# IBM/optimized-number-theoretic-transform-implementations

Measured on AMD Instinct MI355X. Metric: batched forward NTTs/sec at N=2^14, 50-bit q; achieved HBM GB/s vs peak, higher is better.
Workload: dtype f64

## Files before the change

### optimized-number-theoretic-transform-implementations_amd/csrc/ntt_arith.h

```cpp
#pragma once
#include <stdint.h>

#if defined(__HIPCC__)
#  include <hip/hip_runtime.h>
#  define NTT_HD __host__ __device__ __forceinline__
#  define NTT_DEVICE_CODE 1
#else
#  define NTT_HD inline __attribute__((always_inline))
#endif

namespace ntt {

struct alignas(16) TwU64 {
  uint64_t w;
  uint64_t con;
};
struct alignas(16) TwF64 {
  double w;
  double wq;
};

NTT_HD uint64_t mulhi64(uint64_t a, uint64_t b)
{
#if defined(__HIP_DEVICE_COMPILE__)
// ... 238 lines not shown
    const uint64_t p00 = a0 * b0, p01 = a0 * b1, p10 = a1 * b0, p11 = a1 * b1;
    const uint64_t mid = (p00 >> 32) + (uint32_t)p01 + (uint32_t)p10;
    lo                 = (uint32_t)p00 | (mid << 32);
    hi                 = p11 + (p01 >> 32) + (p10 >> 32) + (mid >> 32);
  }
  static NTT_HD uint64_t barrett(uint64_t hi, uint64_t lo, const consts &c)
  {
    const uint64_t q1 = (hi << (64u - c.bsh)) | (lo >> c.bsh);
    return lo - mulhi64(q1, c.bmu) * c.q;
  }
  static constexpr int kDotEvery = K == 3 ? 20 : (K == 1 ? 4 : 1);
  static constexpr int kDotChunk = 2;
  template <bool LAZY> static NTT_HD val dot_term(uint64_t a, uint64_t b, const consts &c)
  {
    if(LAZY && K <= 1) b = csub(b, c.q2);
    if(LAZY && K == 0) a = csub(a, c.q2);
    uint64_t hi, lo;
    mul128(a, b, hi, lo);
    return barrett(hi, lo, c);
  }
  static NTT_HD val dot_acc(val acc, val t, const consts &) { return acc + t; }
  static NTT_HD val dot_fold(val acc, const consts &c) { return reduce_any(acc, c); }
  template <bool LAZY> static NTT_HD val mul_out(val x, uint64_t b, const consts &c)
  {
    if(LAZY && K <= 1) b = csub(b, c.q2);
    if(LAZY && K == 0) b = csub(b, c.q);
    uint64_t hi, lo;
    mul128(reduce_any(x, c), b, hi, lo);
    return barrett(hi, lo, c);
  }
  static NTT_HD uint64_t mul_store(val r, const consts &c) { return csub(csub(r, c.q2), c.q); }
  static NTT_HD uint64_t mul_store_acc(val r, uint64_t acc, const consts &c) { return csub(csub(r + acc, c.q2), c.q); }
};

struct F64Consts {
  double q, qinv;
  double qinv_lo;
  double half_q;
  TwF64  ninv;
  TwF64  wninv;
  uint64_t qi;
  double   q2_sub;
};

struct ArithF64 {
  using val    = double;
  using tw     = TwF64;
  using consts = F64Consts;
  static constexpr bool kTracksBounds = true;
  static constexpr bool kCompact = true;
  static constexpr bool kRadix4  = false;
  static constexpr bool kWide52  = false;
  static constexpr bool kIntWide = false;
  using ctw                      = double;
  static NTT_HD tw expand(ctw w, const consts &c) { return tw{w, fma_(w, c.qinv, w * c.qinv_lo)}; }

  static NTT_HD double magic52() { return 4503599627370496.0; }

  static NTT_HD double u64_to_f64_lt52(uint64_t u)
  {
    union {
      uint64_t u;
      double   d;
    } x;
    x.u = u;
    return __builtin_ldexp(x.d, 1074);
  }
  static NTT_HD double reduce(double v, const consts &c)
  {
    const double k = rint_(v * c.qinv);
    return fma_(-k, c.q, v);
  }
  static NTT_HD double mulmod(const tw &t, double y, const consts &c)
  {
    const double h = y * t.w;
    const double k = rint_(y * t.wq);
    const double l = fma_(y, t.w, -h);
    const double d = fma_(-k, c.q, h);
    return d + l;
  }
  static NTT_HD double mulmod_c(ctw w, double y, const consts &c)
  {
    const double h = y * w;
    const double k = rint_(h * c.qinv);
    const double l = fma_(y, w, -h);
    const double d = fma_(-k, c.q, h);
    return d + l;
  }
  static NTT_HD double mulmod_c2(ctw w, double y, const consts &c)
  {
    const double h = y * w;
    const double k = rint_(fma_(h, c.qinv, h * c.qinv_lo));
    const double l = fma_(y, w, -h);
    const double d = fma_(-k, c.q, h);
    return d + l;
  }
  template <bool INV, bool WIDE> static NTT_HD val load(uint64_t raw, const consts &c)
  {
    if(WIDE) {
      raw = raw < 4 * c.qi ? raw : raw - 4 * c.qi;
      raw = raw < 2 * c.qi ? raw : raw - 2 * c.qi;
      raw = raw < c.qi ? raw : raw - c.qi;
    }
    return u64_to_f64_lt52(raw);
  }
  template <bool RED> static NTT_HD void fwd_bfly(val &x, val &y, const tw &t, const consts &c)
// ... 160 lines not shown
    const double s = x + y;
    const double d = y - x;
    x              = Base::reduce(s, c);
    y              = RED ? Base::mulmod_c(wneg, Base::reduce(d, c), c) : Base::mulmod_c2(wneg, d, c);
  }
  template <bool REDD, bool REDS> static NTT_HD void inv_bfly2(val &x, val &y, const tw &t, const consts &c)
  {
    const double s = x + y;
    const double d = x - y;
    x              = REDS ? Base::reduce(s, c) : s;
    y              = Base::mulmod(t, REDD ? Base::reduce(d, c) : d, c);
  }
  template <bool REDD, bool REDS> static NTT_HD void inv_bfly2(val &x, val &y, ctw w, const consts &c)
  {
    const double s = x + y;
    const double d = x - y;
    x              = REDS ? Base::reduce(s, c) : s;
    y              = REDD ? Base::mulmod_c(w, Base::reduce(d, c), c) : Base::mulmod_c2(w, d, c);
  }
  static NTT_HD void inv_bfly_last(val &x, val &y, const consts &c)
  {
    const double s = Base::reduce(x + y, c);
    const double d = Base::reduce(x - y, c);
    x              = Base::mulmod(c.ninv, s, c);
    y              = Base::mulmod(c.wninv, d, c);
  }
  static NTT_HD uint64_t store_fwd_lazy(val v, const consts &c) { return Base::store_fwd(v, c); }
  static constexpr int kDotEvery = 1;
  static constexpr int kDotChunk = 2;
  template <bool LAZY> static NTT_HD val dot_term(uint64_t a, uint64_t b, const consts &c)
  {
    if(LAZY) {
      a = a < 2 * c.qi ? a : a - 2 * c.qi;
      b = b < 2 * c.qi ? b : b - 2 * c.qi;
    }
    const double x0 = Base::u64_to_f64_lt52(a), y0 = Base::u64_to_f64_lt52(b);
    const double x  = Base::reduce(LAZY ? x0 - c.q : x0, c);
    const double y  = Base::reduce(LAZY ? y0 - c.q : y0, c);
    return Base::mulmod_c(y, x, c);
  }
};
using ArithF64W = WideF64<ArithF64>;

struct ArithF64S {
  using val    = double;
  using tw     = TwF64;
  using consts = F64Consts;
  using ctw    = double;
  static constexpr bool kTracksBounds = true;
  static constexpr bool kCompact      = true;
  static constexpr bool kRadix4       = false;
  static constexpr bool kWide52       = false;
  static constexpr bool kIntWide      = false;
  static NTT_HD tw expand(ctw w, const consts &c) { return ArithF64::expand(w, c); }

  static NTT_HD double word_to_val(uint64_t u)
  {
    union {
      uint64_t u;
      double   d;
    } x;
    x.u = u;
    return x.d;
  }
  static NTT_HD uint64_t val_to_word(double d)
  {
    union {
      double   d;
      uint64_t u;
    } x;
    x.d = d;
    return x.u;
  }
  static NTT_HD double reduce(double v, const consts &c)
  {
    const double k = v * c.qinv;
    return fma_(-k, c.q, v);
  }
  static NTT_HD double mulmod(const tw &t, double y, const consts &c)
  {
    const double h = y * t.w;
    const double k = y * t.wq;
    const double l = fma_(y, t.w, -h);
    const double d = fma_(-k, c.q, h);
    return d + l;
  }
  static NTT_HD double mulmod_c(ctw w, double y, const consts &c)
  {
    const double h = y * w;
    const double k = h * c.qinv;
    const double l = fma_(y, w, -h);
    const double d = fma_(-k, c.q, h);
    return d + l;
  }
  template <bool INV, bool WIDE> static NTT_HD val load(uint64_t raw, const consts &c)
  {
    if(WIDE) {
      raw = raw < 4 * c.qi ? raw : raw - 4 * c.qi;
      raw = raw < 2 * c.qi ? raw : raw - 2 * c.qi;
      raw = raw < c.qi ? raw : raw - c.qi;
    }
    return word_to_val(raw);
  }
  template <bool RED> static NTT_HD void fwd_bfly(val &x, val &y, const tw &t, const consts &c)
  {
    const double xr = RED ? reduce(x, c) : x;
    const double m  = mulmod(t, y, c);
    x               = xr + m;
    y               = xr - m;
  }
  template <bool RED> static NTT_HD void inv_bfly(val &x, val &y, const tw &t, const consts &c)
  {
    const double s = x + y;
    const double d = x - y;
    x              = RED ? reduce(s, c) : s;
    y              = mulmod(t, d, c);
  }
  template <bool RED> static NTT_HD void fwd_bfly(val &x, val &y, ctw w, const consts &c)
  {
    const double xr = RED ? reduce(x, c) : x;
    const double m  = mulmod_c(w, y, c);
    x               = xr + m;
    y               = xr - m;
  }
  template <bool RED> static NTT_HD void inv_bfly(val &x, val &y, ctw w, const consts &c)
  {
    const double s = x + y;
    const double d = x - y;
    x              = RED ? reduce(s, c) : s;
    y              = mulmod_c(w, d, c);
  }
  static NTT_HD void inv_bfly_last(val &x, val &y, const consts &c)
  {
    const double s = x + y;
    const double d = x - y;
    x              = mulmod(c.ninv, s, c);
    y              = mulmod(c.wninv, d, c);
  }
  static NTT_HD uint64_t to_canonical(double v, const consts &c)
  {
    const double   r = reduce(v, c);
    const uint64_t m = c.qi & (uint64_t)((int64_t)val_to_word(r) >> 63);
    return val_to_word(r + word_to_val(m));
  }
  static NTT_HD uint64_t store_fwd(val v, const consts &c) { return to_canonical(v, c); }
  static NTT_HD uint64_t store_inv(val v, const consts &c) { return to_canonical(v, c); }
  static NTT_HD uint64_t store_fwd_lazy(val v, const consts &c) { return val_to_word(v + c.q2_sub); }
  static NTT_HD uint64_t store_inv_lazy(val v, const consts &c) { return to_canonical(v, c); }
  static NTT_HD val      scale_ninv(val v, const consts &c) { return mulmod(c.ninv, v, c); }
};

template <class A> struct scaled_policy {
  using type = A;
};
template <> struct scaled_policy<ArithF64> {
  using type = ArithF64S;
};

struct F64Sched {
  uint32_t mask;
  double   bout;
};

constexpr double f64_rho(double b, double theta2) { return 0.5 + b * theta2 * 1.001 + 0.001; }

constexpr F64Sched f64_schedule_forced(bool inverse, int nstages, int ksh, double b_in, uint32_t cmask, uint32_t force);

constexpr F64Sched f64_schedule(bool inverse, int nstages, int ksh, double b_in, uint32_t cmask = 0, double bout_max = 1e30)
{
  uint32_t force = 0;
  F64Sched sc    = f64_schedule_forced(inverse, nstages, ksh, b_in, cmask, force);
  for(int s = nstages - 1; s >= 0 && sc.bout > bout_max; s--) {
    force |= 1u << s;
    sc = f64_schedule_forced(inverse, nstages, ksh, b_in, cmask, force);
  }
  return sc;
}

constexpr F64Sched f64_schedule_forced(bool inverse, int nstages, int ksh, double b_in, uint32_t cmask, uint32_t force)
{
  double theta2 = 0.25 * 1.001;
  double lim    = 4.0 / 1.001;
  for(int i = 0; i < ksh; i++) {
    theta2 *= 0.5;
    lim *= 2.0;
  }
  lim *= (1.0 - 1.0 / 64.0);
  double   b    = b_in;
  uint32_t mask = 0;
  const double theta2_full = theta2;
  for(int s = 0; s < nstages; s++) {
    theta2 = ((cmask >> s) & 1u) ? 1.5 * theta2_full : theta2_full;
    if(!inverse) {
      const double nr = b + f64_rho(b, theta2);
      if(nr > lim || ((force >> s) & 1u)) {
        mask |= (1u << s);
        b = 0.501 + f64_rho(b, theta2);
      } else {
        b = nr;
      }
    } else {
      const double two_b = 2.0 * b;
      const double r     = f64_rho(two_b, theta2);
      const double nr = two_b > r ? two_b : r;
      if(2.0 * nr > lim) {
        mask |= (1u << s);
        b = r > 0.501 ? r : 0.501;
      } else {
        b = nr;
      }
    }
  }
  return F64Sched{mask, b};
}

constexpr F64Sched f64w_fwd_schedule(int nstages, double b_in, uint32_t cmask)
{
  const double theta2 = 0.5;
  const double lim    = 2.0 * (1.0 - 1.0 / 64.0);
  double       b      = b_in;
  uint32_t     mask   = 0;
  for(int s = 0; s < nstages; s++) {
    const double cc   = ((cmask >> s) & 1u) ? 1.5 : 1.0;
    const double rho  = 0.5 + cc * b * theta2 * 1.001 + 0.001;
    const double ex   = rho + 0.5 * b * theta2 * 1.001;
    const double outb = 0.501 + rho;
    if(ex > lim || outb > lim || b > lim) {
      mask |= 1u << s;
      b = 0.501 + (0.5 + cc * 0.501 * theta2 * 1.001 + 0.001);
    } else {
      b = outb;
    }
  }
  return F64Sched{mask, b};
}

}
```

### optimized-number-theoretic-transform-implementations_amd/csrc/ntt_core.h

```cpp
#pragma once
#include <stdint.h>
#include <type_traits>
#include <utility>

#include "ntt_arith.h"
#include "ntt_passplan.h"

namespace ntt {

constexpr int kLE = 4;
constexpr int kE  = 1 << kLE;

template <int I, int N, class F> NTT_HD void static_for(F &&f)
{
  if constexpr(I < N) {
    f(std::integral_constant<int, I>{});
    static_for<I + 1, N>(f);
  }
}

constexpr int8_t kLaneBits[9][4][6] = {
   {{0, 1, -1, -1, -1, -1}, {2, 3, -1, -1, -1, -1}, {-1, -1, -1, -1, -1, -1}, {-1, -1, -1, -1, -1, -1}},
   {{0, 1, 2, -1, -1, -1}, {5, 6, 0, -1, -1, -1}, {1, 2, 3, -1, -1, -1}, {-1, -1, -1, -1, -1, -1}},
   {{0, 1, 2, 3, -1, -1}, {6, 7, 0, 1, -1, -1}, {2, 3, 4, 5, -1, -1}, {-1, -1, -1, -1, -1, -1}},
// ... 797 lines not shown
  const uint32_t ib = P::IBASE(G, t);
  static_assert(E0 % 2 == 0 && E1 % 2 == 0, "slots come in pairs");
  static_for<E0 / 2, E1 / 2>([&](auto hh) {
    constexpr int E = 2 * decltype(hh)::value;
    const u64x2   v = NT ? stream_load2_nt(coef_at(blk + P::IOFF(G, E), ib)) : stream_load2(coef_at(blk + P::IOFF(G, E), ib));
    raw[E]          = v.a;
    raw[E + 1]      = v.b;
  });
}

template <class A, int LOGN, bool INV>
NTT_HD void global_load_first(typename A::val (&x)[kE], uint32_t t, const uint64_t *blk,
                              bool wide, const typename A::consts &c)
{
  using P = Plan<LOGN>;
  uint64_t raw[kE];
  static_for<0, kE>([&](auto ee) {
    constexpr int   E   = decltype(ee)::value;
    const uint64_t *row = blk + ((uint32_t)E << P::LT);
    raw[E]              = stream_load(coef_at(row, t));
  });
  convert_inputs<A, INV>(x, raw, wide, c);
}

template <class A, int LOGN, bool INV>
NTT_HD void global_load_last(typename A::val (&x)[kE], uint32_t t, const uint64_t *blk,
                             bool wide, const typename A::consts &c)
{
  using P              = Plan<LOGN>;
  constexpr int G      = P::NG - 1;
  const uint32_t ib    = P::IBASE(G, t);
  uint64_t raw[kE];
  static_for<0, kE / 2>([&](auto hh) {
    constexpr int E = 2 * decltype(hh)::value;
    const u64x2   v = stream_load2(coef_at(blk + P::IOFF(G, E), ib));
    raw[E]          = v.a;
    raw[E + 1]      = v.b;
  });
  convert_inputs<A, INV>(x, raw, wide, c);
}

template <class A, bool INV, bool LAZYT> NTT_HD uint64_t out_word(typename A::val v, bool lazy_rt, const typename A::consts &c)
{
  if constexpr(A::kTracksBounds) {
    (void)lazy_rt;
    if constexpr(INV) return A::store_inv(v, c);
    else return LAZYT ? A::store_fwd_lazy(v, c) : A::store_fwd(v, c);
  } else {
    const uint64_t keep = lazy_rt ? 0ull : ~0ull;
    return INV ? A::store_inv_sel(v, c, keep) : A::store_fwd_sel(v, c, keep);
  }
}

template <class A, int LOGN, bool INV, bool LAZYT = false>
NTT_HD void global_store_first(const typename A::val (&x)[kE], uint32_t t, uint64_t *blk,
                               const typename A::consts &c, bool lazy_rt = false)
{
  using P = Plan<LOGN>;
  static_for<0, kE>([&](auto ee) {
    constexpr int E = decltype(ee)::value;
    stream_store(coef_at(blk + ((uint32_t)E << P::LT), t), out_word<A, INV, LAZYT>(x[E], lazy_rt, c));
  });
}

template <class A, int LOGN, bool INV, bool LAZYT = false>
NTT_HD void global_store_last(const typename A::val (&x)[kE], uint32_t t, uint64_t *blk,
                              const typename A::consts &c, bool lazy_rt = false)
{
  using P           = Plan<LOGN>;
  constexpr int G   = P::NG - 1;
  const uint32_t ib = P::IBASE(G, t);
  static_for<0, kE / 2>([&](auto hh) {
    constexpr int E = 2 * decltype(hh)::value;
    u64x2         v;
    v.a = out_word<A, INV, LAZYT>(x[E], lazy_rt, c);
    v.b = out_word<A, INV, LAZYT>(x[E + 1], lazy_rt, c);
    stream_store2(coef_at(blk + P::IOFF(G, E), ib), v);
  });
}

constexpr double kLazyBound = 1.99;

template <class A, int LOGN> constexpr uint32_t fused_cmask()
{
  using P        = Plan<LOGN>;
  uint32_t cmask = 0;
  for(int g = 0; g < P::NG; g++) {
    for(int j = 0; j < P::R(g); j++) {
      if(stage_is_compact<A, LOGN, false>(g, j)) cmask |= 1u << (P::S(g) + j);
    }
  }
  return cmask;
}

template <class A, int LOGN, bool INV, int KSH, bool LAZY = false> constexpr uint32_t fused_mask()
{
  if constexpr(A::kIntWide) {
    return u64x_schedule(INV, LOGN, A::kHead);
  } else if constexpr(!A::kTracksBounds) {
    return 0;
  } else {
    if constexpr(A::kWide52) {
      if constexpr(INV) return 0;
      else return f64w_fwd_schedule(LOGN, 1.0, 0u).mask;
    }
    if constexpr(INV) return kRedPlanFlag | (uint32_t)KSH;
    constexpr F64Sched sc = f64_schedule(false, LOGN, KSH, 1.0, fused_cmask<A, LOGN>(), LAZY ? kLazyBound : 1e30);
    static_assert(!LAZY || sc.bout <= kLazyBound, "lazy forward output: the reduction schedule cannot bound the last stage");
    return sc.mask;
  }
}

template <class A, int R, bool INV, uint32_t MASK>
NTT_HD void column_pass_thread(uint64_t *poly, uint32_t col, uint32_t logn, uint32_t S,
                               bool wide, bool lastinv, const typename A::tw *tab,
                               const typename A::consts &c, bool lazy_out = false)
{
  constexpr int  NE   = 1 << R;
  const uint32_t lsp  = logn - S - R;
  const uint32_t lo   = col & ((1u << lsp) - 1);
  const uint32_t hi   = col >> lsp;
  uint64_t *     base = poly + ((uint64_t)hi << (lsp + R)) + lo;
  typename A::val x[NE];
  static_for<0, NE>([&](auto ee) {
    constexpr int E = decltype(ee)::value;
    const uint64_t r = base[(uint64_t)E << lsp];
    x[E]             = wide ? A::template load<INV, true>(r, c) : A::template load<INV, false>(r, c);
  });
  static_for<0, R>([&](auto jj) {
    constexpr int  J   = INV ? (R - 1 - decltype(jj)::value) : decltype(jj)::value;
    constexpr int  AB  = R - 1 - J;
    constexpr int  POS = INV ? (R - 1 - J) : J;
    constexpr bool RED = (MASK >> POS) & 1u;
    const uint32_t tb  = (1u << (S + J)) + (hi << J);
    static_for<0, NE>([&](auto ee) {
      constexpr int E0 = decltype(ee)::value;
      if constexpr(((E0 >> AB) & 1) == 0) {
        constexpr int E1 = E0 | (1 << AB);
        if(INV && J == 0 && lastinv) {
          A::inv_bfly_last(x[E0], x[E1], c);
        } else {
          const typename A::tw w = tab[tb + (E0 >> (R - J))];
          if constexpr(INV) {
            A::template inv_bfly<RED>(x[E0], x[E1], w, c);
          } else {
            A::template fwd_bfly<RED>(x[E0], x[E1], w, c);
          }
        }
      }
    });
  });
  static_for<0, NE>([&](auto ee) {
    constexpr int E = decltype(ee)::value;
    base[(uint64_t)E << lsp] = out_word<A, INV, false>(x[E], lazy_out, c);
  });
}

template <class A, int R, bool INV>
NTT_HD void column_pass_thread_r4(uint64_t *poly, uint32_t col, uint32_t logn, uint32_t S, const typename A::tw *tab,
                                  const typename A::consts &c, bool lazy_out)
{
// ... 131 lines not shown
```

### optimized-number-theoretic-transform-implementations_amd/csrc/ntt_kernels_block.h

```cpp
#pragma once

namespace ntt {

__device__ __forceinline__ bool below(uint64_t a, uint64_t b) { return (int64_t)(a - b) < 0; }
constexpr int kPreAlso = 12;
constexpr int kIpreMin = 12;

template <class A> constexpr int flavor_of() { return A::kCompact ? 1 : (A::kRadix4 ? 2 : 0); }

template <int LOGN, bool INV, int FLAVOR> struct Geom {
  static constexpr bool COMPACT = FLAVOR == 1 || FLAVOR == 3;
  using P = Plan<LOGN>;
  static constexpr bool PERSIST2 = FLAVOR == 1 && LOGN == 13 && !INV;
  static constexpr int WG  = PERSIST2 ? 1024 : (P::T < 256 ? 256 : P::T);
  static constexpr int BPW = PERSIST2 ? 2 : (P::T < 256 ? 256 / P::T : 1);
  static constexpr bool PERSISTENT = BPW == 1 || PERSIST2;
  static constexpr bool group_is_per_lane(int g)
  {
    for(int j = 0; j < P::R(g); j++)
      if(P::TW_UNIFORM(g, j)) return false;
    return true;
  }
  static constexpr int TBL(int g)
  {
// ... 179 lines not shown
{
  typedef unsigned int v2u32 __attribute__((ext_vector_type(2)));
  const v2u32 v = __builtin_amdgcn_raw_buffer_load_b64(r, (int)voff, (int)soff, AUX);
  return (uint64_t)v.x | ((uint64_t)v.y << 32);
}
template <int AUX = kLoadAux> __device__ __forceinline__ u64x2 buffer_load_u64x2(__amdgpu_buffer_rsrc_t r, uint32_t voff, uint32_t soff)
{
  typedef unsigned int v4u32 __attribute__((ext_vector_type(4)));
  const v4u32 v = __builtin_amdgcn_raw_buffer_load_b128(r, (int)voff, (int)soff, AUX);
  return u64x2{(uint64_t)v.x | ((uint64_t)v.y << 32), (uint64_t)v.z | ((uint64_t)v.w << 32)};
}

template <int LOGN, int AUX = 0>
__device__ __forceinline__ void buffer_store_first_raw(const uint64_t (&u)[kE], uint32_t t, uint64_t *blk)
{
  using P                        = Plan<LOGN>;
  const __amdgpu_buffer_rsrc_t r = block_rsrc<LOGN>(blk);
  typedef unsigned int v2u32 __attribute__((ext_vector_type(2)));
  static_for<0, kE>([&](auto ee) {
    constexpr int E = decltype(ee)::value;
    v2u32         v;
    v.x = (unsigned)u[E];
    v.y = (unsigned)(u[E] >> 32);
    __builtin_amdgcn_raw_buffer_store_b64(v, r, (int)(t * 8u), (int)(((uint32_t)E << P::LT) * 8u), AUX);
  });
}

template <int LOGN, int AUX = kLoadAux>
__device__ __forceinline__ void prefetch_first(uint64_t (&raw)[kE], uint32_t t, const uint64_t *blk, bool live = true)
{
  using P = Plan<LOGN>;
  const __amdgpu_buffer_rsrc_t r = block_rsrc<LOGN>(blk, live);
  static_for<0, kE>([&](auto ee) {
    constexpr int E = decltype(ee)::value;
    raw[E]          = buffer_load_u64<AUX>(r, t * 8u, ((uint32_t)E << P::LT) * 8u);
  });
}

template <int LOGN, int AUX = kLoadAux>
__device__ __forceinline__ void prefetch_last(uint64_t (&raw)[kE], uint32_t t, const uint64_t *blk, bool live = true)
{
  using P           = Plan<LOGN>;
  constexpr int G   = P::NG - 1;
  const uint32_t ib = P::IBASE(G, t);
  const __amdgpu_buffer_rsrc_t r = block_rsrc<LOGN>(blk, live);
  static_for<0, kE / 2>([&](auto hh) {
    constexpr int E = 2 * decltype(hh)::value;
    const u64x2   v = buffer_load_u64x2<AUX>(r, ib * 8u, P::IOFF(G, E) * 8u);
    raw[E]          = v.a;
    raw[E + 1]      = v.b;
  });
}

template <class A, int LOGN, bool LAZYT, int AUX = 0>
__device__ __forceinline__ void store_last_whole_lines(const typename A::val (&x)[kE], uint32_t t, uint64_t *blk,
                                                       const typename A::consts &c, bool lazy_rt)
{
  using P          = Plan<LOGN>;
  constexpr int G  = P::NG - 1;
  constexpr int HB = P::TB(G, 5);
  static_assert(P::RL == 2 && P::NL == 6 && HB > 1, "needs runs of four coefficients per lane and full waves");
  uint64_t u[kE];
  static_for<0, kE>([&](auto ee) { u[decltype(ee)::value] = out_word<A, false, LAZYT>(x[decltype(ee)::value], lazy_rt, c); });
  static_for<0, kE>([&](auto ee) {
    constexpr int E = decltype(ee)::value;
    if constexpr((E & 2) == 0) {
      const auto lo = __builtin_amdgcn_permlane32_swap((unsigned)u[E], (unsigned)u[E | 2], false, false);
      const auto hi = __builtin_amdgcn_permlane32_swap((unsigned)(u[E] >> 32), (unsigned)(u[E | 2] >> 32), false, false);
      u[E]          = (uint64_t)lo[0] | ((uint64_t)hi[0] << 32);
      u[E | 2]      = (uint64_t)lo[1] | ((uint64_t)hi[1] << 32);
    }
  });
  const uint32_t ib   = (P::IBASE(G, t) & ~(1u << HB)) | (((t >> 5) & 1u) << 1);
  const __amdgpu_buffer_rsrc_t r = block_rsrc<LOGN>(blk);
  typedef unsigned int v4u32 __attribute__((ext_vector_type(4)));
  static_for<0, kE / 2>([&](auto hh) {
    constexpr int      E   = 2 * decltype(hh)::value;
    constexpr uint32_t OFF = (P::IOFF(G, E) & ~2u) | ((uint32_t)((E >> 1) & 1) << HB);
    v4u32              v;
    v.x = (unsigned)u[E];
    v.y = (unsigned)(u[E] >> 32);
    v.z = (unsigned)u[E + 1];
    v.w = (unsigned)(u[E + 1] >> 32);
    __builtin_amdgcn_raw_buffer_store_b128(v, r, (int)(ib * 8u), (int)(OFF * 8u), AUX);
  });
}

__device__ __forceinline__ void pin_raw(const uint64_t (&raw)[kE])
{
#pragma unroll
  for(int e = 0; e < kE; e++) asm volatile("" ::"v"(raw[e]));
}
template <class A, int LOGN, int G>
__device__ __forceinline__ void pin_preloaded(const typename A::ctw (&pre)[4][kE / 2])
{
  using P = Plan<LOGN>;
#pragma unroll
  for(int j = 0; j < P::R(G); j++) {
#pragma unroll
    for(int b = 0; b < kE / 2; b++) {
      if(P::BFLY_FIRST(G, j, b) == b) asm volatile("" ::"v"(pre[j][b]));
    }
  }
}

template <class A, int LOGN, bool INV, class G = Geom<LOGN, INV, flavor_of<A>()>>
__device__ __forceinline__ void fill_lds_tables(typename A::ctw *tabl, const Params<A> &p, uint32_t blk0, uint32_t tid)
{
  using P = Plan<LOGN>;
  static_for<0, P::NG>([&](auto gg) {
    constexpr int GI = decltype(gg)::value;
    if constexpr(G::TBL(GI) > 0) {
      typename A::ctw *tg = tabl + G::TBL_OFF(GI);
      static_for<0, P::R(GI)>([&](auto jj) {
        constexpr int JJ  = decltype(jj)::value;
        constexpr int SG  = P::S(GI);
        constexpr int SLJ = SG + JJ;
        const typename A::ctw *src = p.tw8 + ((size_t)1 << (p.s0 + SLJ)) + ((size_t)blk0 << SLJ);
        for(uint32_t l = tid; l < (1u << SLJ); l += G::WG) {
          const uint32_t u = l & ((1u << JJ) - 1u), prefix = l >> JJ;
          tg[(((1u << JJ) - 1u) << SG) + (u << SG) + prefix] = src[l];
        }
      });
    }
  });
}

template <class AK, int LOGN, bool INV, int KSH, bool LASTINV = false, bool LAZY = false, bool MULTI = false>
__global__ void __launch_bounds__((Geom<LOGN, INV, flavor_of<AK>()>::WG), (Geom<LOGN, INV, flavor_of<AK>()>::WPS)) fused_kernel(const KArgs<AK> k)
{
  using A = typename scaled_policy<AK>::type;
  uint32_t        bid, gdim, limb_;
  const Params<A> p = limb_params<A, INV, MULTI>(k, bid, gdim, limb_);
  using P                 = Plan<LOGN>;
  using G                 = Geom<LOGN, INV, flavor_of<A>()>;
  static_assert(!LAZY || (!INV && A::kTracksBounds), "the LAZY variant exists for the FP64 forward kernels only");
  constexpr uint32_t MASK = fused_mask<A, LOGN, INV, KSH, LAZY>() | (INV && LASTINV ? kLastInvFlag : 0u) | (INV && A::kWide52 ? kCanonInFlag : 0u);
  constexpr int LDS_TW = G::LDS_TW;
  __shared__ typename A::val lds_all[G::BPW * P::LDS_ELEMS + LDS_TW];

  const uint32_t     tid = threadIdx.x;
  const uint32_t     sub = G::PERSIST2 ? uniform_u32(tid >> P::LT) : (tid >> P::LT);
  const uint32_t     t   = tid & (P::T - 1);
  typename A::val *  lds = lds_all + sub * P::LDS_ELEMS;
  const uint32_t     bmask = (1u << p.s0) - 1u;

  if constexpr(!INV && G::PERSISTENT && !A::kRadix4) {
    constexpr int  GL     = P::NG - 1;
    constexpr bool PRE    = A::kCompact && (LOGN == 14 || LOGN == 13 || LOGN == kPreAlso) && stage_is_compact<A, LOGN, false>(GL, 0) && G::TBL(GL) == 0;
    constexpr bool LTW    = LDS_TW > 0;
    const uint32_t         tt     = G::BPW == 1 ? tid : t;
    typename A::val *const ll     = G::BPW == 1 ? lds_all : lds;
    const uint64_t         stride = (uint64_t)gdim * G::BPW;
    uint64_t               b0     = (uint64_t)bid * G::BPW;
    if(b0 >= p.nblocks) return;
    const uint64_t lastb = p.nblocks - 1;
    uint64_t       b     = G::BPW == 1 ? b0 : (b0 + sub < p.nblocks ? b0 + sub : lastb);
    typename A::ctw *const tabl = reinterpret_cast<typename A::ctw *>(lds_all + G::BPW * P::LDS_ELEMS);
    const lds_ctw_ptr<A>   ltw  = (lds_ctw_ptr<A>)tabl;
    if constexpr(LTW) {
      fill_lds_tables<A, LOGN, INV>(tabl, p, (uint32_t)b & bmask, tid);
      __syncthreads();
    }
    const auto next_blk = [&](uint64_t at) -> uint64_t {
      const uint64_t n0 = below(at + stride, p.nblocks) ? at + stride : at;
      return G::BPW == 1 ? n0 : (n0 + sub < p.nblocks ? n0 + sub : lastb);
    };
    uint64_t off_cur = blk_off_t<LOGN>(p, b), off_nxt = blk_off_t<LOGN>(p, next_blk(b0));
    uint64_t raw[kE];
    prefetch_first<LOGN>(raw, tt, p.a + off_cur);
    pin_raw(raw);
    typename A::ctw pre[4][kE / 2];
    if constexpr(PRE) {
      preload_group_tw<A, LOGN, GL>(pre, tt, (uint32_t)b & bmask, p);
      pin_preloaded<A, LOGN, GL>(pre);
    }
    for(; b0 < p.nblocks; b0 += stride) {
      const bool live = G::BPW == 1 || b0 + sub < p.nblocks;
      b               = live ? b0 + (G::BPW == 1 ? 0u : sub) : lastb;
      const uint32_t blk  = (uint32_t)b & bmask;
      uint64_t *     base = p.a + off_cur;
      typename A::val x[kE];
      convert_inputs<A, false>(x, raw, p.wide != 0, p.c);
      {
        const bool     more = b0 + stride < p.nblocks;
        prefetch_first<LOGN>(raw, tt, p.a + off_nxt, more);
        off_cur = off_nxt;
        off_nxt = blk_off_t<LOGN>(p, next_blk(more ? b0 + stride : b0));
      }
      run_group<A, LOGN, 0, false, MASK>(x, tt, blk, p);
      static_for<0, P::NG - 1>([&](auto gg) {
        constexpr int GI = decltype(gg)::value;
        exchange<A, LOGN, GI, GI + 1>(x, tt, ll);
        if constexpr(PRE && GI + 1 == GL) {
          run_group_preloaded<A, LOGN, GL, MASK>(x, pre, p);
        } else if constexpr(G::TBL(GI + 1) > 0) {
          run_group<A, LOGN, GI + 1, false, MASK, true>(x, tt, blk, p, ltw + G::TBL_OFF(GI + 1));
        } else {
          run_group<A, LOGN, GI + 1, false, MASK>(x, tt, blk, p);
        }
      });
      if constexpr(LOGN == 14) {
        store_last_whole_lines<A, LOGN, LAZY>(x, tid, base, p.c, p.lazy != 0);
      } else {
        if(live) global_store_last<A, LOGN, false, LAZY>(x, tt, base, p.c, p.lazy != 0);
      }
    }
    return;
  }
  if constexpr(INV && G::PERSISTENT && A::kCompact) {
    constexpr int  GL     = P::NG - 1;
    constexpr bool LTW    = LDS_TW > 0;
    const uint32_t         tt     = G::BPW == 1 ? tid : t;
    typename A::val *const ll     = G::BPW == 1 ? lds_all : lds;
    const uint64_t         stride = (uint64_t)gdim * G::BPW;
    uint64_t               b0     = (uint64_t)bid * G::BPW;
    if(b0 >= p.nblocks) return;
    const uint64_t lastb = p.nblocks - 1;
    uint64_t       b     = G::BPW == 1 ? b0 : (b0 + sub < p.nblocks ? b0 + sub : lastb);
    typename A::ctw *const tabl = reinterpret_cast<typename A::ctw *>(lds_all + G::BPW * P::LDS_ELEMS);
    const lds_ctw_ptr<A>   ltw  = (lds_ctw_ptr<A>)tabl;
    if constexpr(LTW) {
      fill_lds_tables<A, LOGN, INV>(tabl, p, (uint32_t)b & bmask, tid);
      __syncthreads();
    }
    constexpr bool IPRE = A::kCompact && LOGN >= kIpreMin && stage_is_compact<A, LOGN, true>(GL, 0) && P::R(GL) < 4 && G::TBL(GL) == 0 &&
                          !(LOGN == 12 && KSH == 1);
    typename A::ctw pre[4][kE / 2];
    if constexpr(IPRE) preload_group_tw<A, LOGN, GL>(pre, tt, (uint32_t)b & bmask, p);
    const auto next_blk = [&](uint64_t at) -> uint64_t {
      const uint64_t n0 = below(at + stride, p.nblocks) ? at + stride : at;
      return G::BPW == 1 ? n0 : (n0 + sub < p.nblocks ? n0 + sub : lastb);
    };
    uint64_t off_cur = blk_off_t<LOGN>(p, b), off_nxt = blk_off_t<LOGN>(p, next_blk(b0));
    uint64_t raw[kE];
    prefetch_last<LOGN>(raw, tt, p.a + off_cur);
    pin_raw(raw);
    if constexpr(IPRE) pin_preloaded<A, LOGN, GL>(pre);
    for(; b0 < p.nblocks; b0 += stride) {
      const bool live = G::BPW == 1 || b0 + sub < p.nblocks;
      b               = live ? b0 + (G::BPW == 1 ? 0u : sub) : lastb;
      const uint32_t blk  = (uint32_t)b & bmask;
      uint64_t *     base = p.a + off_cur;
      typename A::val x[kE];
      convert_inputs<A, true>(x, raw, p.wide != 0, p.c);
      {
        const bool     more = b0 + stride < p.nblocks;
        prefetch_last<LOGN>(raw, tt, p.a + off_nxt, more);
        off_cur = off_nxt;
        off_nxt = blk_off_t<LOGN>(p, next_blk(more ? b0 + stride : b0));
      }
      if constexpr(IPRE) {
        run_group_preloaded<A, LOGN, GL, MASK, true>(x, pre, p);
      } else if constexpr(G::TBL(GL) > 0) {
        run_group<A, LOGN, GL, true, MASK, true>(x, tt, blk, p, ltw + G::TBL_OFF(GL));
      } else {
        run_group<A, LOGN, GL, true, MASK>(x, tt, blk, p);
      }
      static_for<0, P::NG - 1>([&](auto gg) {
        constexpr int GI = P::NG - 1 - decltype(gg)::value;
        exchange<A, LOGN, GI, GI - 1>(x, tt, ll);
        if constexpr(G::TBL(GI - 1) > 0) {
          run_group<A, LOGN, GI - 1, true, MASK, true>(x, tt, blk, p, ltw + G::TBL_OFF(GI - 1));
        } else {
          run_group<A, LOGN, GI - 1, true, MASK>(x, tt, blk, p);
        }
      });
      uint64_t out[kE];
      static_for<0, kE>([&](auto ee) { out[decltype(ee)::value] = A::store_inv(x[decltype(ee)::value], p.c); });
      if(live) buffer_store_first_raw<LOGN>(out, tt, base);
    }
    return;
  }

  const lds_ctw_ptr<A> gtw = (lds_ctw_ptr<A>)reinterpret_cast<typename A::ctw *>(lds_all + G::BPW * P::LDS_ELEMS);
  if constexpr(LDS_TW > 0) {
    fill_lds_tables<A, LOGN, INV>(reinterpret_cast<typename A::ctw *>(lds_all + G::BPW * P::LDS_ELEMS), p, 0u, tid);
    __syncthreads();
  }
  for(uint64_t b0 = (uint64_t)bid * G::BPW; b0 < p.nblocks; b0 += (uint64_t)gdim * G::BPW) {
    uint64_t   b    = b0 + sub;
    const bool live = b < p.nblocks;
    if(!live) b = p.nblocks - 1;
    const uint32_t blk  = (uint32_t)b & bmask;
    uint64_t *     base = p.a + (poly_offset<false>(b >> p.s0, p.pstride, p.ptab) + ((b & bmask) << LOGN));
    typename A::val x[kE];
    if constexpr(!INV) {
      global_load_first<A, LOGN, false>(x, t, base, p.wide != 0, p.c);
      run_group<A, LOGN, 0, false, MASK, (G::TBL(0) > 0)>(x, t, blk, p, gtw);
      static_for<0, P::NG - 1>([&](auto gg) {
        constexpr int GI = decltype(gg)::value;
        exchange<A, LOGN, GI, GI + 1>(x, t, lds);
        run_group<A, LOGN, GI + 1, false, MASK, (G::TBL(GI + 1) > 0)>(x, t, blk, p, gtw + G::TBL_OFF(GI + 1));
      });
      if(live) global_store_last<A, LOGN, false, LAZY>(x, t, base, p.c, p.lazy != 0);
    } else {
      global_load_last<A, LOGN, true>(x, t, base, p.wide != 0, p.c);
      run_group<A, LOGN, P::NG - 1, true, MASK, (G::TBL(P::NG - 1) > 0)>(x, t, blk, p, gtw + G::TBL_OFF(P::NG - 1));
      static_for<0, P::NG - 1>([&](auto gg) {
        constexpr int GI = P::NG - 1 - decltype(gg)::value;
        exchange<A, LOGN, GI, GI - 1>(x, t, lds);
        run_group<A, LOGN, GI - 1, true, MASK, (G::TBL(GI - 1) > 0)>(x, t, blk, p, gtw + G::TBL_OFF(GI - 1));
      });
      if(live) global_store_first<A, LOGN, true>(x, t, base, p.c, p.lazy != 0);
    }
  }
}

template <int LEAD> __device__ __forceinline__ __amdgpu_buffer_rsrc_t poly_rsrc(const uint64_t *poly)
{
  return __builtin_amdgcn_make_buffer_rsrc(const_cast<uint64_t *>(poly), 0, (int)(8u << (kFusedLarge + LEAD)), 0x00020000);
}

template <class A, int LEAD, bool INV, int KSH>
__device__ __forceinline__ void twophase_columns(uint64_t *base, uint32_t tid, const Params<A> &p, bool wide_in, bool lazy_out)
{
  constexpr int      NE    = 1 << LEAD;
  constexpr int      CPR   = kE / NE;
  constexpr int      NR    = kE / CPR;
  constexpr uint32_t CMASK = column_mask<A, LEAD, INV, KSH>();
  const __amdgpu_buffer_rsrc_t r = poly_rsrc<LEAD>(base);
  typedef unsigned int v2u32 __attribute__((ext_vector_type(2)));
  uint64_t raw[kE];
  auto load_round = [&](auto rr, uint64_t(&dst)[kE]) {
    constexpr int RD = decltype(rr)::value;
    static_for<0, kE>([&](auto vv) {
      constexpr int      V   = decltype(vv)::value;
      constexpr uint32_t OFF = ((uint32_t)(V % NE) << kFusedLarge) + (uint32_t)(RD * CPR + V / NE) * 1024u;
      dst[V]                 = buffer_load_u64(r, tid * 8u, OFF * 8u);
    });
  };
  load_round(std::integral_constant<int, 0>{}, raw);
  static_for<0, NR>([&](auto rr) {
    constexpr int RD = decltype(rr)::value;
    typename A::val x[kE];
    convert_inputs<A, INV>(x, raw, wide_in, p.c);
    if constexpr(RD + 1 < NR) load_round(std::integral_constant<int, RD + 1>{}, raw);
    static_for<0, LEAD>([&](auto jj) {
      constexpr int  J   = INV ? (LEAD - 1 - decltype(jj)::value) : decltype(jj)::value;
      constexpr int  AB  = LEAD - 1 - J;
      constexpr int  POS = INV ? (LEAD - 1 - J) : J;
      constexpr bool RED = (CMASK >> POS) & 1u;
      static_for<0, kE>([&](auto vv) {
        constexpr int V  = decltype(vv)::value;
        constexpr int E0 = V % NE;
        if constexpr(((E0 >> AB) & 1) == 0) {
          constexpr int V1 = V | (1 << AB);
          if constexpr(INV && J == 0) {
// ... 391 lines not shown
```

Baseline: 19.92 million.

## Offset forward FP64 scaled outputs by half-q to drop final canonicalization select

For the scaled FP64 forward kernel, subtracts (q-1)/2 (in scaled representation) from coefficient 0 of the input. Since the NTT is linear, this shifts every output by that constant, so the final store can use a single reduce plus add of the offset instead of reduce, sign mask and conditional add. The reduction schedule gains per-policy constants (tighter for the scaled policy) and a relaxed output bound, which may remove intermediate reduction stages. This relies on the offset keeping results in [0,q) and on the bound analysis being correct.

```diff
diff --git a/optimized-number-theoretic-transform-implementations_amd/csrc/ntt_arith.h b/optimized-number-theoretic-transform-implementations_amd/csrc/ntt_arith.h
--- a/optimized-number-theoretic-transform-implementations_amd/csrc/ntt_arith.h
+++ b/optimized-number-theoretic-transform-implementations_amd/csrc/ntt_arith.h
@@ -314,6 +314,7 @@
   static constexpr bool kRadix4  = false;
   static constexpr bool kWide52  = false;
   static constexpr bool kIntWide = false;
+  static constexpr double kSchedFull = 1.0, kSchedCompact = 1.5;
   using ctw                      = double;
   static NTT_HD tw expand(ctw w, const consts &c) { return tw{w, fma_(w, c.qinv, w * c.qinv_lo)}; }
 
@@ -580,6 +581,7 @@
   static constexpr bool kRadix4       = false;
   static constexpr bool kWide52       = false;
   static constexpr bool kIntWide      = false;
+  static constexpr double kSchedFull = 0.5, kSchedCompact = 1.0;
   static NTT_HD tw expand(ctw w, const consts &c) { return ArithF64::expand(w, c); }
 
   static NTT_HD double word_to_val(uint64_t u)
@@ -673,6 +675,8 @@
   }
   static NTT_HD uint64_t store_fwd(val v, const consts &c) { return to_canonical(v, c); }
   static NTT_HD uint64_t store_inv(val v, const consts &c) { return to_canonical(v, c); }
+  static NTT_HD double   half_off(const consts &c) { return word_to_val((c.qi - 1u) >> 1); }
+  static NTT_HD uint64_t store_fwd_off(val v, double hoff, const consts &c) { return val_to_word(reduce(v, c) + hoff); }
   static NTT_HD uint64_t store_fwd_lazy(val v, const consts &c) { return val_to_word(v + c.q2_sub); }
   static NTT_HD uint64_t store_inv_lazy(val v, const consts &c) { return to_canonical(v, c); }
   static NTT_HD val      scale_ninv(val v, const consts &c) { return mulmod(c.ninv, v, c); }
@@ -692,20 +696,22 @@
 
 constexpr double f64_rho(double b, double theta2) { return 0.5 + b * theta2 * 1.001 + 0.001; }
 
-constexpr F64Sched f64_schedule_forced(bool inverse, int nstages, int ksh, double b_in, uint32_t cmask, uint32_t force);
-
-constexpr F64Sched f64_schedule(bool inverse, int nstages, int ksh, double b_in, uint32_t cmask = 0, double bout_max = 1e30)
+constexpr F64Sched f64_schedule_forced(bool inverse, int nstages, int ksh, double b_in, uint32_t cmask, uint32_t force, double cf = 1.0,
+                                       double cc = 1.5);
+
+constexpr F64Sched f64_schedule(bool inverse, int nstages, int ksh, double b_in, uint32_t cmask = 0, double bout_max = 1e30, double cf = 1.0,
+                                double cc = 1.5)
 {
   uint32_t force = 0;
-  F64Sched sc    = f64_schedule_forced(inverse, nstages, ksh, b_in, cmask, force);
+  F64Sched sc    = f64_schedule_forced(inverse, nstages, ksh, b_in, cmask, force, cf, cc);
   for(int s = nstages - 1; s >= 0 && sc.bout > bout_max; s--) {
     force |= 1u << s;
-    sc = f64_schedule_forced(inverse, nstages, ksh, b_in, cmask, force);
+    sc = f64_schedule_forced(inverse, nstages, ksh, b_in, cmask, force, cf, cc);
   }
   return sc;
 }
 
-constexpr F64Sched f64_schedule_forced(bool inverse, int nstages, int ksh, double b_in, uint32_t cmask, uint32_t force)
+constexpr F64Sched f64_schedule_forced(bool inverse, int nstages, int ksh, double b_in, uint32_t cmask, uint32_t force, double cf, double cc)
 {
   double theta2 = 0.25 * 1.001;
   double lim    = 4.0 / 1.001;
@@ -718,7 +724,7 @@
   uint32_t mask = 0;
   const double theta2_full = theta2;
   for(int s = 0; s < nstages; s++) {
-    theta2 = ((cmask >> s) & 1u) ? 1.5 * theta2_full : theta2_full;
+    theta2 = (((cmask >> s) & 1u) ? cc : cf) * theta2_full;
     if(!inverse) {
       const double nr = b + f64_rho(b, theta2);
       if(nr > lim || ((force >> s) & 1u)) {
diff --git a/optimized-number-theoretic-transform-implementations_amd/csrc/ntt_core.h b/optimized-number-theoretic-transform-implementations_amd/csrc/ntt_core.h
--- a/optimized-number-theoretic-transform-implementations_amd/csrc/ntt_core.h
+++ b/optimized-number-theoretic-transform-implementations_amd/csrc/ntt_core.h
@@ -873,6 +873,23 @@
   }
 }
 
+template <class A> NTT_HD void fwd_offset_input(typename A::val (&x)[kE], bool first, typename A::val hoff)
+{
+  if(first) x[0] = x[0] - hoff;
+}
+template <class A, bool INV, bool LAZYT, bool OFFS>
+NTT_HD uint64_t out_word_off(typename A::val v, bool lazy_rt, typename A::val hoff, const typename A::consts &c)
+{
+  if constexpr(OFFS) {
+    static_assert(!INV && !LAZYT, "offset outputs: the canonical forward output only");
+    (void)lazy_rt;
+    return A::store_fwd_off(v, hoff, c);
+  } else {
+    (void)hoff;
+    return out_word<A, INV, LAZYT>(v, lazy_rt, c);
+  }
+}
+
 template <class A, int LOGN, bool INV, bool LAZYT = false>
 NTT_HD void global_store_first(const typename A::val (&x)[kE], uint32_t t, uint64_t *blk,
                                const typename A::consts &c, bool lazy_rt = false)
@@ -884,9 +901,9 @@
   });
 }
 
-template <class A, int LOGN, bool INV, bool LAZYT = false>
+template <class A, int LOGN, bool INV, bool LAZYT = false, bool OFFS = false>
 NTT_HD void global_store_last(const typename A::val (&x)[kE], uint32_t t, uint64_t *blk,
-                              const typename A::consts &c, bool lazy_rt = false)
+                              const typename A::consts &c, bool lazy_rt = false, typename A::val hoff = {})
 {
   using P           = Plan<LOGN>;
   constexpr int G   = P::NG - 1;
@@ -894,8 +911,8 @@
   static_for<0, kE / 2>([&](auto hh) {
     constexpr int E = 2 * decltype(hh)::value;
     u64x2         v;
-    v.a = out_word<A, INV, LAZYT>(x[E], lazy_rt, c);
-    v.b = out_word<A, INV, LAZYT>(x[E + 1], lazy_rt, c);
+    v.a = out_word_off<A, INV, LAZYT, OFFS>(x[E], lazy_rt, hoff, c);
+    v.b = out_word_off<A, INV, LAZYT, OFFS>(x[E + 1], lazy_rt, hoff, c);
     stream_store2(coef_at(blk + P::IOFF(G, E), ib), v);
   });
 }
@@ -914,8 +931,9 @@
   return cmask;
 }
 
-template <class A, int LOGN, bool INV, int KSH, bool LAZY = false> constexpr uint32_t fused_mask()
-{
+template <class A, int LOGN, bool INV, int KSH, bool LAZY = false, bool OFFS = false> constexpr uint32_t fused_mask()
+{
+  static_assert(!OFFS || (!INV && !LAZY && A::kTracksBounds && !A::kWide52), "offset outputs: the canonical forward output of the FP64 policy");
   if constexpr(A::kIntWide) {
     return u64x_schedule(INV, LOGN, A::kHead);
   } else if constexpr(!A::kTracksBounds) {
@@ -926,8 +944,10 @@
       else return f64w_fwd_schedule(LOGN, 1.0, 0u).mask;
     }
     if constexpr(INV) return kRedPlanFlag | (uint32_t)KSH;
-    constexpr F64Sched sc = f64_schedule(false, LOGN, KSH, 1.0, fused_cmask<A, LOGN>(), LAZY ? kLazyBound : 1e30);
+    constexpr double   bmax = LAZY ? kLazyBound : (OFFS ? kLazyBound * (double)(1u << (KSH < 31 ? KSH : 31)) : 1e30);
+    constexpr F64Sched sc   = f64_schedule(false, LOGN, KSH, 1.0, fused_cmask<A, LOGN>(), bmax, A::kSchedFull, A::kSchedCompact);
     static_assert(!LAZY || sc.bout <= kLazyBound, "lazy forward output: the reduction schedule cannot bound the last stage");
+    static_assert(!OFFS || sc.bout <= bmax, "offset forward output: the reduction schedule cannot keep the last stage below 2^52");
     return sc.mask;
   }
 }
diff --git a/optimized-number-theoretic-transform-implementations_amd/csrc/ntt_kernels_block.h b/optimized-number-theoretic-transform-implementations_amd/csrc/ntt_kernels_block.h
--- a/optimized-number-theoretic-transform-implementations_amd/csrc/ntt_kernels_block.h
+++ b/optimized-number-theoretic-transform-implementations_amd/csrc/ntt_kernels_block.h
@@ -255,16 +255,16 @@
   });
 }
 
-template <class A, int LOGN, bool LAZYT, int AUX = 0>
+template <class A, int LOGN, bool LAZYT, int AUX = 0, bool OFFS = false>
 __device__ __forceinline__ void store_last_whole_lines(const typename A::val (&x)[kE], uint32_t t, uint64_t *blk,
-                                                       const typename A::consts &c, bool lazy_rt)
+                                                       const typename A::consts &c, bool lazy_rt, typename A::val hoff = {})
 {
   using P          = Plan<LOGN>;
   constexpr int G  = P::NG - 1;
   constexpr int HB = P::TB(G, 5);
   static_assert(P::RL == 2 && P::NL == 6 && HB > 1, "needs runs of four coefficients per lane and full waves");
   uint64_t u[kE];
-  static_for<0, kE>([&](auto ee) { u[decltype(ee)::value] = out_word<A, false, LAZYT>(x[decltype(ee)::value], lazy_rt, c); });
+  static_for<0, kE>([&](auto ee) { u[decltype(ee)::value] = out_word_off<A, false, LAZYT, OFFS>(x[decltype(ee)::value], lazy_rt, hoff, c); });
   static_for<0, kE>([&](auto ee) {
     constexpr int E = decltype(ee)::value;
     if constexpr((E & 2) == 0) {
@@ -338,7 +338,8 @@
   using P                 = Plan<LOGN>;
   using G                 = Geom<LOGN, INV, flavor_of<A>()>;
   static_assert(!LAZY || (!INV && A::kTracksBounds), "the LAZY variant exists for the FP64 forward kernels only");
-  constexpr uint32_t MASK = fused_mask<A, LOGN, INV, KSH, LAZY>() | (INV && LASTINV ? kLastInvFlag : 0u) | (INV && A::kWide52 ? kCanonInFlag : 0u);
+  constexpr bool     OFFS = !INV && !LAZY && std::is_same<A, ArithF64S>::value;
+  constexpr uint32_t MASK = fused_mask<A, LOGN, INV, KSH, LAZY, OFFS>() | (INV && LASTINV ? kLastInvFlag : 0u) | (INV && A::kWide52 ? kCanonInFlag : 0u);
   constexpr int LDS_TW = G::LDS_TW;
   __shared__ typename A::val lds_all[G::BPW * P::LDS_ELEMS + LDS_TW];
 
@@ -378,6 +379,9 @@
       preload_group_tw<A, LOGN, GL>(pre, tt, (uint32_t)b & bmask, p);
       pin_preloaded<A, LOGN, GL>(pre);
     }
+    typename A::val hoff{};
+    if constexpr(OFFS) hoff = A::half_off(p.c);
+    const bool first = tt == 0;
     for(; b0 < p.nblocks; b0 += stride) {
       const bool live = G::BPW == 1 || b0 + sub < p.nblocks;
       b               = live ? b0 + (G::BPW == 1 ? 0u : sub) : lastb;
@@ -385,6 +389,7 @@
       uint64_t *     base = p.a + off_cur;
       typename A::val x[kE];
       convert_inputs<A, false>(x, raw, p.wide != 0, p.c);
+      if constexpr(OFFS) fwd_offset_input<A>(x, first, hoff);
       {
         const bool     more = b0 + stride < p.nblocks;
         prefetch_first<LOGN>(raw, tt, p.a + off_nxt, more);
@@ -404,9 +409,9 @@
         }
       });
       if constexpr(LOGN == 14) {
-        store_last_whole_lines<A, LOGN, LAZY>(x, tid, base, p.c, p.lazy != 0);
+        store_last_whole_lines<A, LOGN, LAZY, 0, OFFS>(x, tid, base, p.c, p.lazy != 0, hoff);
       } else {
-        if(live) global_store_last<A, LOGN, false, LAZY>(x, tt, base, p.c, p.lazy != 0);
+        if(live) global_store_last<A, LOGN, false, LAZY, OFFS>(x, tt, base, p.c, p.lazy != 0, hoff);
       }
     }
     return;
@@ -481,6 +486,9 @@
     fill_lds_tables<A, LOGN, INV>(reinterpret_cast<typename A::ctw *>(lds_all + G::BPW * P::LDS_ELEMS), p, 0u, tid);
     __syncthreads();
   }
+  typename A::val hoff{};
+  if constexpr(OFFS) hoff = A::half_off(p.c);
+  const bool first = t == 0;
   for(uint64_t b0 = (uint64_t)bid * G::BPW; b0 < p.nblocks; b0 += (uint64_t)gdim * G::BPW) {
     uint64_t   b    = b0 + sub;
     const bool live = b < p.nblocks;
@@ -490,13 +498,14 @@
     typename A::val x[kE];
     if constexpr(!INV) {
       global_load_first<A, LOGN, false>(x, t, base, p.wide != 0, p.c);
+      if constexpr(OFFS) fwd_offset_input<A>(x, first, hoff);
       run_group<A, LOGN, 0, false, MASK, (G::TBL(0) > 0)>(x, t, blk, p, gtw);
       static_for<0, P::NG - 1>([&](auto gg) {
         constexpr int GI = decltype(gg)::value;
         exchange<A, LOGN, GI, GI + 1>(x, t, lds);
         run_group<A, LOGN, GI + 1, false, MASK, (G::TBL(GI + 1) > 0)>(x, t, blk, p, gtw + G::TBL_OFF(GI + 1));
       });
-      if(live) global_store_last<A, LOGN, false, LAZY>(x, t, base, p.c, p.lazy != 0);
+      if(live) global_store_last<A, LOGN, false, LAZY, OFFS>(x, t, base, p.c, p.lazy != 0, hoff);
     } else {
       global_load_last<A, LOGN, true>(x, t, base, p.wide != 0, p.c);
       run_group<A, LOGN, P::NG - 1, true, MASK, (G::TBL(P::NG - 1) > 0)>(x, t, blk, p, gtw + G::TBL_OFF(P::NG - 1));
```

New measurement: 20.05 million, median of 6. About the same (+0.6%).

## Fold canonical output correction into an injected DC offset and refine F64S bound schedule

Applied to the files above, without the earlier changes.

For the scaled FP64 forward kernel, a constant offset of (q-1)/2 is subtracted from coefficient 0 before the transform. Because the forward NTT spreads a DC term evenly to every output, each output can then be made canonical with a single reduce plus add, with no sign-mask correction. The bound schedule now takes per-arithmetic rho factors, using tighter ones for ArithF64S, and caps the final bound at half the class limit. The aim is fewer instructions per stored word and possibly fewer intermediate reductions, at the cost of relying on tighter numerical bound reasoning.

```diff
diff --git a/optimized-number-theoretic-transform-implementations_amd/csrc/ntt_arith.h b/optimized-number-theoretic-transform-implementations_amd/csrc/ntt_arith.h
--- a/optimized-number-theoretic-transform-implementations_amd/csrc/ntt_arith.h
+++ b/optimized-number-theoretic-transform-implementations_amd/csrc/ntt_arith.h
@@ -314,6 +314,7 @@
   static constexpr bool kRadix4  = false;
   static constexpr bool kWide52  = false;
   static constexpr bool kIntWide = false;
+  static constexpr double kRhoFull = 1.0, kRhoCompact = 1.5;
   using ctw                      = double;
   static NTT_HD tw expand(ctw w, const consts &c) { return tw{w, fma_(w, c.qinv, w * c.qinv_lo)}; }
 
@@ -580,6 +581,7 @@
   static constexpr bool kRadix4       = false;
   static constexpr bool kWide52       = false;
   static constexpr bool kIntWide      = false;
+  static constexpr double kRhoFull = 0.5, kRhoCompact = 1.0;
   static NTT_HD tw expand(ctw w, const consts &c) { return ArithF64::expand(w, c); }
 
   static NTT_HD double word_to_val(uint64_t u)
@@ -673,6 +675,9 @@
   }
   static NTT_HD uint64_t store_fwd(val v, const consts &c) { return to_canonical(v, c); }
   static NTT_HD uint64_t store_inv(val v, const consts &c) { return to_canonical(v, c); }
+  static NTT_HD double   off_c0(const consts &c) { return word_to_val((c.qi - 1) >> 1); }
+  static NTT_HD val      off_inject(val v, const consts &c) { return v - off_c0(c); }
+  static NTT_HD uint64_t store_fwd_off(val v, const consts &c) { return val_to_word(reduce(v, c) + off_c0(c)); }
   static NTT_HD uint64_t store_fwd_lazy(val v, const consts &c) { return val_to_word(v + c.q2_sub); }
   static NTT_HD uint64_t store_inv_lazy(val v, const consts &c) { return to_canonical(v, c); }
   static NTT_HD val      scale_ninv(val v, const consts &c) { return mulmod(c.ninv, v, c); }
@@ -692,20 +697,30 @@
 
 constexpr double f64_rho(double b, double theta2) { return 0.5 + b * theta2 * 1.001 + 0.001; }
 
-constexpr F64Sched f64_schedule_forced(bool inverse, int nstages, int ksh, double b_in, uint32_t cmask, uint32_t force);
-
-constexpr F64Sched f64_schedule(bool inverse, int nstages, int ksh, double b_in, uint32_t cmask = 0, double bout_max = 1e30)
+constexpr F64Sched f64_schedule_forced(bool inverse, int nstages, int ksh, double b_in, uint32_t cmask, uint32_t force, double rho_full = 1.0,
+                                       double rho_compact = 1.5);
+
+constexpr F64Sched f64_schedule(bool inverse, int nstages, int ksh, double b_in, uint32_t cmask = 0, double bout_max = 1e30, double rho_full = 1.0,
+                                double rho_compact = 1.5)
 {
   uint32_t force = 0;
-  F64Sched sc    = f64_schedule_forced(inverse, nstages, ksh, b_in, cmask, force);
+  F64Sched sc    = f64_schedule_forced(inverse, nstages, ksh, b_in, cmask, force, rho_full, rho_compact);
   for(int s = nstages - 1; s >= 0 && sc.bout > bout_max; s--) {
     force |= 1u << s;
-    sc = f64_schedule_forced(inverse, nstages, ksh, b_in, cmask, force);
+    sc = f64_schedule_forced(inverse, nstages, ksh, b_in, cmask, force, rho_full, rho_compact);
   }
   return sc;
 }
 
-constexpr F64Sched f64_schedule_forced(bool inverse, int nstages, int ksh, double b_in, uint32_t cmask, uint32_t force)
+constexpr double f64_class_limit(int ksh)
+{
+  double lim = 4.0 / 1.001;
+  for(int i = 0; i < ksh; i++) lim *= 2.0;
+  return lim * (1.0 - 1.0 / 64.0);
+}
+
+constexpr F64Sched f64_schedule_forced(bool inverse, int nstages, int ksh, double b_in, uint32_t cmask, uint32_t force, double rho_full,
+                                       double rho_compact)
 {
   double theta2 = 0.25 * 1.001;
   double lim    = 4.0 / 1.001;
@@ -718,7 +733,7 @@
   uint32_t mask = 0;
   const double theta2_full = theta2;
   for(int s = 0; s < nstages; s++) {
-    theta2 = ((cmask >> s) & 1u) ? 1.5 * theta2_full : theta2_full;
+    theta2 = (((cmask >> s) & 1u) ? rho_compact : rho_full) * theta2_full;
     if(!inverse) {
       const double nr = b + f64_rho(b, theta2);
       if(nr > lim || ((force >> s) & 1u)) {
diff --git a/optimized-number-theoretic-transform-implementations_amd/csrc/ntt_core.h b/optimized-number-theoretic-transform-implementations_amd/csrc/ntt_core.h
--- a/optimized-number-theoretic-transform-implementations_amd/csrc/ntt_core.h
+++ b/optimized-number-theoretic-transform-implementations_amd/csrc/ntt_core.h
@@ -873,6 +873,27 @@
   }
 }
 
+#ifndef NTT_OFFSET_OUT
+#  define NTT_OFFSET_OUT 1
+#endif
+template <class A, bool INV, bool LAZY> constexpr bool fused_offset_out() { return NTT_OFFSET_OUT && !INV && !LAZY && std::is_base_of<ArithF64S, A>::value; }
+
+template <class A> NTT_HD void inject_offset(typename A::val (&x)[kE], uint32_t t, const typename A::consts &c)
+{
+  if(t == 0) x[0] = A::off_inject(x[0], c);
+}
+
+template <class A, bool INV, bool LAZYT, bool OFF> NTT_HD uint64_t out_word_sel(typename A::val v, bool lazy_rt, const typename A::consts &c)
+{
+  if constexpr(OFF) {
+    static_assert(!INV && !LAZYT, "offset outputs: canonical forward words only");
+    (void)lazy_rt;
+    return A::store_fwd_off(v, c);
+  } else {
+    return out_word<A, INV, LAZYT>(v, lazy_rt, c);
+  }
+}
+
 template <class A, int LOGN, bool INV, bool LAZYT = false>
 NTT_HD void global_store_first(const typename A::val (&x)[kE], uint32_t t, uint64_t *blk,
                                const typename A::consts &c, bool lazy_rt = false)
@@ -884,7 +905,7 @@
   });
 }
 
-template <class A, int LOGN, bool INV, bool LAZYT = false>
+template <class A, int LOGN, bool INV, bool LAZYT = false, bool OFF = false>
 NTT_HD void global_store_last(const typename A::val (&x)[kE], uint32_t t, uint64_t *blk,
                               const typename A::consts &c, bool lazy_rt = false)
 {
@@ -894,8 +915,8 @@
   static_for<0, kE / 2>([&](auto hh) {
     constexpr int E = 2 * decltype(hh)::value;
     u64x2         v;
-    v.a = out_word<A, INV, LAZYT>(x[E], lazy_rt, c);
-    v.b = out_word<A, INV, LAZYT>(x[E + 1], lazy_rt, c);
+    v.a = out_word_sel<A, INV, LAZYT, OFF>(x[E], lazy_rt, c);
+    v.b = out_word_sel<A, INV, LAZYT, OFF>(x[E + 1], lazy_rt, c);
     stream_store2(coef_at(blk + P::IOFF(G, E), ib), v);
   });
 }
@@ -926,7 +947,10 @@
       else return f64w_fwd_schedule(LOGN, 1.0, 0u).mask;
     }
     if constexpr(INV) return kRedPlanFlag | (uint32_t)KSH;
-    constexpr F64Sched sc = f64_schedule(false, LOGN, KSH, 1.0, fused_cmask<A, LOGN>(), LAZY ? kLazyBound : 1e30);
+    constexpr bool   OFF  = fused_offset_out<A, INV, LAZY>();
+    constexpr double BMAX = LAZY ? kLazyBound : (OFF ? 0.5 * f64_class_limit(KSH) : 1e30);
+    constexpr F64Sched sc = f64_schedule(false, LOGN, KSH, 1.0, fused_cmask<A, LOGN>(), BMAX, A::kRhoFull, A::kRhoCompact);
+    static_assert(!OFF || sc.bout <= BMAX, "offset forward output: the reduction schedule cannot bound the last stage");
     static_assert(!LAZY || sc.bout <= kLazyBound, "lazy forward output: the reduction schedule cannot bound the last stage");
     return sc.mask;
   }
diff --git a/optimized-number-theoretic-transform-implementations_amd/csrc/ntt_kernels_block.h b/optimized-number-theoretic-transform-implementations_amd/csrc/ntt_kernels_block.h
--- a/optimized-number-theoretic-transform-implementations_amd/csrc/ntt_kernels_block.h
+++ b/optimized-number-theoretic-transform-implementations_amd/csrc/ntt_kernels_block.h
@@ -255,7 +255,7 @@
   });
 }
 
-template <class A, int LOGN, bool LAZYT, int AUX = 0>
+template <class A, int LOGN, bool LAZYT, int AUX = 0, bool OFFSET = false>
 __device__ __forceinline__ void store_last_whole_lines(const typename A::val (&x)[kE], uint32_t t, uint64_t *blk,
                                                        const typename A::consts &c, bool lazy_rt)
 {
@@ -264,7 +264,7 @@
   constexpr int HB = P::TB(G, 5);
   static_assert(P::RL == 2 && P::NL == 6 && HB > 1, "needs runs of four coefficients per lane and full waves");
   uint64_t u[kE];
-  static_for<0, kE>([&](auto ee) { u[decltype(ee)::value] = out_word<A, false, LAZYT>(x[decltype(ee)::value], lazy_rt, c); });
+  static_for<0, kE>([&](auto ee) { u[decltype(ee)::value] = out_word_sel<A, false, LAZYT, OFFSET>(x[decltype(ee)::value], lazy_rt, c); });
   static_for<0, kE>([&](auto ee) {
     constexpr int E = decltype(ee)::value;
     if constexpr((E & 2) == 0) {
@@ -339,6 +339,7 @@
   using G                 = Geom<LOGN, INV, flavor_of<A>()>;
   static_assert(!LAZY || (!INV && A::kTracksBounds), "the LAZY variant exists for the FP64 forward kernels only");
   constexpr uint32_t MASK = fused_mask<A, LOGN, INV, KSH, LAZY>() | (INV && LASTINV ? kLastInvFlag : 0u) | (INV && A::kWide52 ? kCanonInFlag : 0u);
+  constexpr bool OFF = fused_offset_out<A, INV, LAZY>();
   constexpr int LDS_TW = G::LDS_TW;
   __shared__ typename A::val lds_all[G::BPW * P::LDS_ELEMS + LDS_TW];
 
@@ -385,6 +386,7 @@
       uint64_t *     base = p.a + off_cur;
       typename A::val x[kE];
       convert_inputs<A, false>(x, raw, p.wide != 0, p.c);
+      if constexpr(OFF) inject_offset<A>(x, tt, p.c);
       {
         const bool     more = b0 + stride < p.nblocks;
         prefetch_first<LOGN>(raw, tt, p.a + off_nxt, more);
@@ -404,9 +406,9 @@
         }
       });
       if constexpr(LOGN == 14) {
-        store_last_whole_lines<A, LOGN, LAZY>(x, tid, base, p.c, p.lazy != 0);
+        store_last_whole_lines<A, LOGN, LAZY, 0, OFF>(x, tid, base, p.c, p.lazy != 0);
       } else {
-        if(live) global_store_last<A, LOGN, false, LAZY>(x, tt, base, p.c, p.lazy != 0);
+        if(live) global_store_last<A, LOGN, false, LAZY, OFF>(x, tt, base, p.c, p.lazy != 0);
       }
     }
     return;
@@ -490,13 +492,14 @@
     typename A::val x[kE];
     if constexpr(!INV) {
       global_load_first<A, LOGN, false>(x, t, base, p.wide != 0, p.c);
+      if constexpr(OFF) inject_offset<A>(x, t, p.c);
       run_group<A, LOGN, 0, false, MASK, (G::TBL(0) > 0)>(x, t, blk, p, gtw);
       static_for<0, P::NG - 1>([&](auto gg) {
         constexpr int GI = decltype(gg)::value;
         exchange<A, LOGN, GI, GI + 1>(x, t, lds);
         run_group<A, LOGN, GI + 1, false, MASK, (G::TBL(GI + 1) > 0)>(x, t, blk, p, gtw + G::TBL_OFF(GI + 1));
       });
-      if(live) global_store_last<A, LOGN, false, LAZY>(x, t, base, p.c, p.lazy != 0);
+      if(live) global_store_last<A, LOGN, false, LAZY, OFF>(x, t, base, p.c, p.lazy != 0);
     } else {
       global_load_last<A, LOGN, true>(x, t, base, p.wide != 0, p.c);
       run_group<A, LOGN, P::NG - 1, true, MASK, (G::TBL(P::NG - 1) > 0)>(x, t, blk, p, gtw + G::TBL_OFF(P::NG - 1));
```

Measured after the change: 20.10 million before, 20.08 million after. Within noise of the previous version (-0.1%).
